# filrg/distributed_cluster_GPUs

Measured on AMD Instinct MI355X. Metric: sim_events_per_sec, higher is better.
Workload: dtype fp64; 1 GPU; model=paper_config multi-DC geo-cluster DES, global_batch=4096, seq_len=4000, parallelism=replica_shard_dp1, algo=default_policy, replicas_per_gpu=4096, arrivals=sinusoid inf 6/s amp 0.6 period 300 + poisson trn 0.3/s, fp32_coeff_eval=False, topology=8 DC / 1488 GPUs / 8 ingresses

## Files before the change

distributed_cluster_gpus_amd/engine/batched.py:

```python
import math
import os
from typing import Optional

import numpy as np
import torch

from ..models.arrivals import ArrivalProcess
from ..models.scenario import Scenario
from ..ops import load_sim_hip
from ..utils.csvlog import ClusterLogWriter, JobLogWriter
from ..utils.timers import ThroughputMeter
from .oracle import ALGOS
from .state import (INF, RL_HID, SERIES_METRICS, alloc_state, engine_cfg,
                    engine_dims, load_tensors)

SERIES_FLEET = "ALL"


class BatchedEngine:
    def __init__(self, scenario: Scenario,
                 arrival_inf: ArrivalProcess, arrival_trn: ArrivalProcess,
                 *, algo: str = "default_policy", replicas: int = 4096,
                 duration: float = 3600.0, log_interval: float = 10.0,
                 out_dir: Optional[str] = None, seed: int = 42,
                 power_cap: float = 0.0, control_interval: float = 5.0,
                 elastic_scaling: bool = False, eco_objective: str = "energy",
                 num_fixed_gpus: int = 1, fixed_freq: Optional[float] = None,
                 logger=None, show_progress: bool = False,
                 device: Optional[torch.device] = None,
# ... 1 lines not shown
                 tcap: int = 64, qcap: int = 24576,
                 events_per_launch: int = 50000,
                 enable_logs: bool = True,
                 sla_p99_ms: float = 500.0, energy_budget_j=None,
                 rl_device: str = 'cuda', rl_batch: int = 256,
                 rl_warmup: int = 1000, rl_buffer: int = 200000,
                 rl_train_interval: int = 256, rl_agent=None,
                 rl_stats_interval: int = 100,
                 rl_serve: str = "device", rl_deterministic: bool = False,
                 rl_exact_p99: bool = False, fp32_coeff_eval: bool = False,
                 rl_tr_limit: Optional[int] = None, rl_reserve_cus: int = 16,
                 rl_target_updates_per_s: float = 180.0,
                 tr_cap: int = 262144, arrival_trace=None,
                 subwave: int = 64,
                 pop_series: bool = False, pop_series_every: int = 1,
                 **_unused):
        if algo not in ALGOS:
            raise ValueError(f"unknown algo {algo!r}")
        if pop_series and int(pop_series_every) < 1:
            raise ValueError("pop_series_every must be >= 1")
        if not torch.cuda.is_available():
            raise RuntimeError("BatchedEngine requires a ROCm GPU "
                               "(no silent CPU fallback)")
        self._mod = load_sim_hip("_sim_hip" if subwave == 64 else "_sim_hip_mw")
        self.sc = scenario
        self.algo = algo
        self.device = device or torch.device("cuda", torch.cuda.current_device())
        self.end_time = float(duration)
        self.log_interval = float(log_interval)
        self.events_per_launch = int(events_per_launch)
# ... 67 lines not shown
                and not self._rl_det

        dims = engine_dims(
            scenario, algo=algo, n_rep=R, duration=duration,
            log_interval=log_interval, tcap=tcap, qcap=qcap,
            events_per_launch=events_per_launch,
            log_replica=self.log_replica,
            pop_series_every=self.pop_series_every,
            arrival_trace=arrival_trace, power_cap=power_cap,
            eco_objective=eco_objective, fp32_coeff_eval=fp32_coeff_eval,
            num_fixed_gpus=num_fixed_gpus, fixed_freq=fixed_freq, seed=seed,
            rep_id_offset=shard.start, sla_p99_ms=sla_p99_ms, tr_cap=tr_cap,
            elastic_scaling=elastic_scaling, rl_exact_p99=rl_exact_p99,
            serve_device=self._serve_device, weights_buffer=self._mfma_serve,
            rl_deterministic=rl_deterministic, rl_tr_limit=rl_tr_limit,
            rl_train_interval=rl_train_interval)
        self.dims = dims
        if self.pop_series:
            ps_bytes = dims.ps_cap * (n_dc + 1) * len(SERIES_METRICS) * R * 8
            import logging
            from ..utils.logging import LOGGER_NAME
            (logger or logging.getLogger(LOGGER_NAME)).info(
                f"pop_series: sample buffer {dims.ps_cap} ticks x {n_dc + 1} "
                f"rows x {len(SERIES_METRICS)} metrics x {R} replicas x 8 B = "
                f"{ps_bytes} bytes ({ps_bytes / 2**20:.1f} MiB)")
        t = alloc_state(dims, scenario, dev, arrival_trace)
        if not self.trace_mode:
            arr_np = self._seed_arrivals(arrival_inf, arrival_trn, seed, shard)
            t["arr_next"].copy_(torch.as_tensor(arr_np, dtype=torch.float64))
        self.t = t
        self.arrival_inf, self.arrival_trn = arrival_inf, arrival_trn
# ... 501 lines not shown
```

distributed_cluster_gpus_amd/engine/state.py:

```python
import math
from dataclasses import dataclass
from typing import Optional

import numpy as np
import torch

from ..models.scenario import PAYLOAD_GB, Scenario

ALGO_IDS = {"default_policy": 0, "cap_uniform": 1, "cap_greedy": 2,
            "joint_nf": 3, "bandit": 4, "carbon_cost": 5, "eco_route": 6,
            "debug": 7, "chsac_af": 8}
ECO_IDS = {"energy": 0, "carbon": 1, "cost": 2}
MODE_IDS = {"poisson": 0, "sinusoid": 1, "off": 2}
INF = 1e300
SERIES_METRICS = ("freq", "busy", "running", "q_inf", "q_trn", "power_w",
                  "energy_j")
RL_HID = 256
P99_WIN = 2048


@dataclass(frozen=True)
class EngineDims:
    algo: str
    n_rep: int
    n_dc: int
    n_ing: int
    n_freq: int
    total_slots: int
    tcap: int
    qcap: int
    end_time: float
    log_interval: float
    log_replica: int
# ... 8 lines not shown
    fp32_score: int
    num_fixed: int
    fixed_freq: float
    seed: int
    rep_id_offset: int
    sla_p99_ms: float
    obs_dim: int
    tr_cap: int
    pp_cap: int
    elastic: int
    exact_p99: int
    serve_device: int
    weights_numel: int
    rl_det: int
    tr_limit: int

    @property
    def is_rl(self) -> bool:
        return self.algo == "chsac_af"

    @property
    def n_streams(self) -> int:
        return self.n_ing * 2


def policy_weights_numel(obs_dim: int, n_dc: int, n_g: int,
                         hid: int = RL_HID) -> int:
    H = hid
    return (obs_dim * H + H) + 2 * (H * H + H) + (H * H + H) + \
        (H * n_dc + n_dc) + (H * H + H) + (H * n_g + n_g)


def engine_dims(scenario: Scenario, *, algo: str, n_rep: int,
                duration: float = 3600.0, log_interval: float = 10.0,
                tcap: int = 64, qcap: int = 24576,
                events_per_launch: int = 50000, log_replica: int = -1,
                pop_series_every: int = 0, arrival_trace=None,
                power_cap: float = 0.0, eco_objective: str = "energy",
                fp32_coeff_eval: bool = False, num_fixed_gpus: int = 1,
                fixed_freq: Optional[float] = None, seed: int = 42,
                rep_id_offset: int = 0, sla_p99_ms: float = 500.0,
                tr_cap: int = 262144, elastic_scaling: bool = False,
                rl_exact_p99: bool = False, serve_device: bool = False,
                weights_buffer: bool = False, rl_deterministic: bool = False,
                rl_tr_limit: Optional[int] = None,
                rl_train_interval: int = 256) -> EngineDims:
    is_rl = algo == "chsac_af"
    n_dc = scenario.n_dc
    end_time, log_interval = float(duration), float(log_interval)
    n_ticks = int(math.ceil(end_time / log_interval))
    logs = log_replica >= 0
    obs_dim = 1 + 6 * n_dc
    n_g = int(scenario.policy.max_gpus_per_job)
    tr_cap = int(tr_cap) if is_rl else 0
    tr_limit = int(rl_tr_limit) if rl_tr_limit is not None else \
        min(tr_cap // 2, int(rl_train_interval) * 256)
    return EngineDims(
        algo=algo, n_rep=int(n_rep), n_dc=n_dc, n_ing=scenario.n_ing,
        n_freq=scenario.n_freq,
        total_slots=int(scenario.total_gpus.sum()), tcap=int(tcap),
        qcap=int(qcap), end_time=end_time, log_interval=log_interval,
        log_replica=int(log_replica),
        cl_cap=(n_dc * (n_ticks + 2) + 64) if logs else 1,
        jl_cap=max(65536, 2 * int(events_per_launch)) if logs else 1,
        ps_every=int(pop_series_every),
        ps_cap=(n_ticks // int(pop_series_every) + 2) if pop_series_every
        else 0,
        trace_mode=arrival_trace is not None,
        trace_cap=int(np.asarray(arrival_trace[0]).shape[2])
        if arrival_trace is not None else 0,
        power_cap=float(power_cap), eco_obj=ECO_IDS[eco_objective],
        fp32_score=int(bool(fp32_coeff_eval)), num_fixed=int(num_fixed_gpus),
        fixed_freq=float(fixed_freq) if fixed_freq else 0.0,
        seed=int(seed), rep_id_offset=int(rep_id_offset),
        sla_p99_ms=float(sla_p99_ms),
        obs_dim=obs_dim, tr_cap=tr_cap,
        pp_cap=int(scenario.total_gpus.max()) if is_rl else 0,
        elastic=int(bool(elastic_scaling) and is_rl),
        exact_p99=int(bool(rl_exact_p99) and is_rl),
        serve_device=int(bool(serve_device) and is_rl),
        weights_numel=policy_weights_numel(obs_dim, n_dc, n_g)
        if (is_rl and (serve_device or weights_buffer)) else 1,
        rl_det=int(bool(rl_deterministic) and is_rl),
        tr_limit=tr_limit if is_rl else 0)


def alloc_state(dims: EngineDims, scenario: Scenario, device,
                arrival_trace=None) -> dict:
    d = dims
    dev = torch.device(device)
    R, n_dc, n_freq, NS = d.n_rep, d.n_dc, d.n_freq, d.n_streams
    total_slots, tcap, qcap = d.total_slots, d.tcap, d.qcap
    f64 = dict(dtype=torch.float64, device=dev)
    f32 = dict(dtype=torch.float32, device=dev)
    i64 = dict(dtype=torch.int64, device=dev)
    i32 = dict(dtype=torch.int32, device=dev)
    i16 = dict(dtype=torch.int16, device=dev)
    i8 = dict(dtype=torch.int8, device=dev)
    u8 = dict(dtype=torch.uint8, device=dev)
# ... 71 lines not shown
    t["jobs_done_inf"] = torch.zeros(R, **i64)
    t["sum_lat"] = torch.zeros(R, **f64)
    t["sum_lat_inf"] = torch.zeros(R, **f64)
    t["sum_wait"] = torch.zeros(R, **f64)
    t["cl_count"] = torch.zeros(1, **i32)
    t["cl_rows"] = torch.zeros((d.cl_cap, 15), **f64)
    t["jl_count"] = torch.zeros(1, **i32)
    t["jl_rows"] = torch.zeros((d.jl_cap, 11), **f64)

    if d.ps_every:
        t["ps_samples"] = torch.zeros(
            (d.ps_cap, n_dc + 1, len(SERIES_METRICS), R), **f64)
        t["ps_time"] = torch.zeros(d.ps_cap, **f64)
        t["ps_tick"] = torch.zeros(R, **i32)

    if d.trace_mode:
        tt, ts = arrival_trace[0], arrival_trace[1]
        td = arrival_trace[2] if len(arrival_trace) > 2 else \
            np.full(np.asarray(tt).shape, -1, np.int8)
        tt = np.asarray(tt, np.float64)
        ts = np.asarray(ts, np.float64)
        td = np.asarray(td, np.int8)
        assert tt.shape == (R, NS, d.trace_cap), tt.shape
        t["trace_time"] = T(tt)
        t["trace_size"] = T(ts)
        t["trace_dc"] = T(td)
        t["trace_pos"] = torch.zeros((R, NS), **i32)
        t["arr_next"].copy_(t["trace_time"][:, :, 0])

    if d.is_rl:
# ... 83 lines not shown
        "fp32_score": d.fp32_score, "num_fixed": d.num_fixed,
        "fixed_freq": d.fixed_freq,
        "payload_inf_gb": PAYLOAD_GB[0], "payload_trn_gb": PAYLOAD_GB[1],
        "arr_mode": [MODE_IDS[arrival_inf.mode], MODE_IDS[arrival_trn.mode]],
        "arr_rate": [float(arrival_inf.rate), float(arrival_trn.rate)],
        "arr_amp": [float(arrival_inf.amp), float(arrival_trn.amp)],
        "arr_period": [float(arrival_inf.period), float(arrival_trn.period)],
        "seed": d.seed, "rep_id_offset": d.rep_id_offset,
        "log_replica": d.log_replica, "cl_cap": d.cl_cap, "jl_cap": d.jl_cap,
        "obs_dim": d.obs_dim, "sla_p99_ms": d.sla_p99_ms, "tr_cap": d.tr_cap,
        "elastic": d.elastic, "pp_cap": d.pp_cap,
        "trace_mode": int(d.trace_mode), "trace_cap": d.trace_cap,
        "serve_device": d.serve_device, "rl_hid": RL_HID, "rl_det": d.rl_det,
        "tr_limit": d.tr_limit, "exact_p99": d.exact_p99,
        "p99_win": P99_WIN, "pop_series_every": d.ps_every,
    }
```

distributed_cluster_gpus_amd/ops/csrc/hip/engine_bind.hpp:

```cpp
#pragma once
#include <torch/extension.h>

#include <string>
#include <tuple>
#include <type_traits>
#include <unordered_map>
#include <vector>

#include "engine_desc.hpp"

namespace dcg {

template <class T> struct ElemOf;
#define DCG_ELEM(T, ST) \
  template <> struct ElemOf<T> { static constexpr auto dtype = torch::ST; }
DCG_ELEM(double, kFloat64);
DCG_ELEM(float, kFloat32);
DCG_ELEM(int, kInt32);
DCG_ELEM(short, kInt16);
DCG_ELEM(char, kInt8);
DCG_ELEM(unsigned char, kUInt8);
DCG_ELEM(long long, kInt64);
DCG_ELEM(uint64_t, kInt64);
DCG_ELEM(SRec, kFloat64);
DCG_ELEM(XRec, kFloat64);
#undef DCG_ELEM

class Binder {
 public:
  using Row = std::tuple<std::string, std::string, int64_t>;

  explicit Binder(const std::unordered_map<std::string, torch::Tensor>& t)
      : t_(t) {}

  template <class P>
  void operator()(P*& field, const char* name, int64_t need) {
    using E = std::remove_const_t<P>;
    const auto dtype = ElemOf<E>::dtype;
    const int64_t item = (int64_t)c10::elementSize(dtype);
    const int64_t per = (int64_t)sizeof(E) / item;
// ... 45 lines not shown
```

distributed_cluster_gpus_amd/ops/csrc/hip/engine_desc.hpp:

```cpp
#pragma once
#include <cstddef>
#include <cstdint>

namespace dcg {

constexpr int MAX_DC = 8;
constexpr int MAX_FREQ = 8;

struct XRec {
  double size;
  float netlat;
  int jid;
  short nsel;
  unsigned char dc, jtype, ing, adc, ag, mdc;
  unsigned char mg, has_rl, pad0, pad1;
};
static_assert(sizeof(XRec) == 32, "XRec must be one 32B record");

struct SRec {
  double start, lastupd, size, fused, done;
  float netlat;
  int jid;
  int seq;
  unsigned char ing, pcount, nrew, adc, ag, mdc, mg, has_rl;
  unsigned char pad[4];
};
static_assert(sizeof(SRec) == 64, "SRec must be one 64B record");

enum Algo { A_DEFAULT = 0, A_CAP_UNIFORM, A_CAP_GREEDY, A_JOINT_NF, A_BANDIT,
            A_CARBON_COST, A_ECO_ROUTE, A_DEBUG, A_CHSAC };

enum PendKind : int { PEND_NONE = 0, PEND_ARRIVAL = 1, PEND_DRAIN = 2,
                      PEND_REALLOC = 3 };
enum ReqFlag : int { REQ_IDLE = 0, REQ_PENDING = 1, REQ_READY = 2 };

constexpr int LAT_BINS = 64;

enum Err : int { ERR_NONE = 0, ERR_QUEUE_OVF = 1, ERR_XFER_OVF = 2,
                 ERR_SLOT_OVF = 4, ERR_LOG_OVF = 8 };

constexpr int MAX_STREAMS = 16;
constexpr int RL_MAX_HID = 256;
constexpr int RL_MAX_OBS = 64;
constexpr int RL_MAX_LOG = 16;

struct EngineDesc {
  int n_rep, n_dc, n_ing, n_freq, n_streams, total_slots, tcap, qcap;
  double end_time, log_interval;
  const double* freq_levels;
  const double* pc;
  const double* lc;
  const double* wan_lat;
  const double* wan_bw;
  const double* carbon;
// ... 119 lines not shown
  int p99_win;
  double* p99_sorted;
  double* p99_ring;
  int tr_cap;
  int* tr_count;
  float* tr_s0;
  float* tr_s1;
  unsigned char* tr_adc;
  unsigned char* tr_ag;
  float* tr_r;
  float* tr_costs;
  unsigned char* tr_mdc;
  unsigned char* tr_mg;
};

static_assert(sizeof(SRec) == 8 * sizeof(double), "s_rec rows are 8 f64 wide");
static_assert(sizeof(XRec) == 4 * sizeof(double), "x_rec rows are 4 f64 wide");

}
```

distributed_cluster_gpus_amd/ops/csrc/hip/replica_engine.hip:

```cpp
#include <torch/extension.h>
#include <ATen/hip/HIPContext.h>
#include <hip/hip_runtime.h>

#include <cstdint>
#include <cstdlib>
#include <string>
#include <tuple>
#include <unordered_map>
#include <vector>

#include "engine_bind.hpp"
#include "engine_desc.hpp"
#include "engine_limits.hpp"
#include "launch_plan.hpp"
#include "philox.hpp"
#include "pop_series.hpp"
#include "sim_models.hpp"

namespace dcg {

__device__ __forceinline__ void store_fence() {
  asm volatile("s_waitcnt vmcnt(0) lgkmcnt(0)" ::: "memory");
}

__device__ __forceinline__ void lds_fence() {
// ... 337 lines not shown

__device__ double draw_interarrival(Ctx& c, int jt, double t) {
  const EngineDesc& S = *c.S;
  double rate = S.arr_rate[jt];
  int mode = S.arr_mode[jt];
  double amp = S.arr_amp[jt];
  double period = S.arr_period[jt];
  double ia = D_INF;
  if (mode == 0 && rate > 0) {
    ia = rexp(c.rng, rate);
  } else if (mode == 1) {
    double max_rate = rate * (1.0 + fabs(amp));
    if (max_rate > 0) {
      for (int it = 0; it < 4096; ++it) {
        double w = rexp(c.rng, max_rate);
        double lam = fmax(0.0, rate * (1.0 + amp *
            sin(2.0 * M_PI * fmod(t + w, period) / period)));
        if (u01(c.rng) <= lam / max_rate) { ia = w; break; }
      }
    }
  }
  return ia;
}

__device__ void push_transfer(Ctx& c, double now, int jt, int ing, double size,
                              int jid, int d_sel,
                              const JobTrace* tr = nullptr) {
  const EngineDesc& S = *c.S;
  double lnet = launch_const(S.wan_lat)[ing * S.n_dc + d_sel];
  double bw = launch_const(S.wan_bw)[ing * S.n_dc + d_sel];
  double xfer = bw > 0.0 ? S.payload_gb[jt] / bw : 0.0;
  int cand = sub_first_empty(c.l_xt, 0, S.tcap);
// ... 698 lines not shown
    rl_serve_inline(c, now, a_dc, a_g, mdc, mg);
    rl_realloc_entry(c, cur, a_g, mdc, mg, now);
  }
  if (c.lane == 0) {
    S.pp_count[c.r] = 0;
    S.pp_cursor[c.r] = 0;
  }
  store_fence();
}

#if DCG_SUBWAVE == 8
#define DCG_ADVANCE_BOUNDS __launch_bounds__(THREADS_PER_BLOCK, 2)
#else
#define DCG_ADVANCE_BOUNDS __launch_bounds__(THREADS_PER_BLOCK)
#endif
template <int ALGO, bool PS, bool WIN>
__global__ void DCG_ADVANCE_BOUNDS
advance_kernel(EngineDesc S, double t_target, long long max_ev,
               PopSeriesDesc P, LaunchWindow W) {
  int slot_id = sub_uniform_i32((blockIdx.x * blockDim.x + threadIdx.x) / SUBW);
  int lane = threadIdx.x & (SUBW - 1);
  static_assert(!(WIN && ALGO == A_CHSAC), "chsac has no windowed kernel");
  if (slot_id >= (WIN ? W.count : S.n_rep)) return;
  long long ev_skip = 0;
  if (WIN) {
    slot_id += W.first;
    if (slot_id >= S.n_rep) slot_id -= S.n_rep;
    slot_id = sub_uniform_i32(slot_id);
    ev_skip = sub_uniform_i64(
        (blockIdx.x * blockDim.x + threadIdx.x) / SUBW >= W.split
            ? W.ev_a - W.ev_b : 0ll);
  }

  Ctx c;
  c.S = &S;
  c.r = slot_id;
  c.lane = lane;
  if (S.done[c.r]) return;
  if (ALGO == A_CHSAC && S.pend_kind[c.r] != PEND_NONE &&
      S.req_flag[c.r] != REQ_READY)
    return;
  c.now = S.now[c.r];
  {
    bool own = lane < S.n_dc;
    c.my_total = own ? S.total_gpus[lane] : 0;
    c.my_pidle = own ? (S.power_gating[lane] ? S.p_sleep[lane]
                                             : S.p_idle[lane]) : 0.0;
  }
  c.rng.key = S.seed ^ (0x9E3779B97F4A7C15ull * (uint64_t)(S.rep_id_offset + c.r));
  c.rng.ctr = S.rng_ctr[c.r];

  const int NS = S.n_streams;
  int64_t sbase = (int64_t)c.r * S.total_slots;
  long long n_events = ev_skip;
  bool paused = false;
  bool skip_loop = false;

  extern __shared__ __attribute__((aligned(16))) char smem[];
  {
    const LdsSizes z = lds_sizes(S.total_slots, S.tcap, ALGO == A_CHSAC);
    char* base = smem + (threadIdx.x / SUBW) * z.stride();
    c.hs = reinterpret_cast<Hot*>(base);
    if (SUBW == 64) {
      c.l_fin = reinterpret_cast<double*>(base + z.hot);
      c.l_xt = reinterpret_cast<double*>(base + z.hot + z.fin);
// ... 160 lines not shown
      break;
    }
    if (t_min > t_target) break;

    accrue_to(c, t_min);
    c.now = t_min;
    n_events++;

    if (kind == 0) {
      int ing = idx >> 1;
      int jt = idx & 1;
      int jid = c.hs->jid_ctr + 1;
      if (lane == 0) c.hs->jid_ctr = jid;
      double size;
      int trace_d = -1;
      if (S.trace_mode) {
        int64_t tb = ((int64_t)c.r * S.n_streams + idx) * S.trace_cap;
        int posn = S.trace_pos[(int64_t)c.r * S.n_streams + idx];
        size = S.trace_size[tb + posn];
        trace_d = S.trace_dc[tb + posn];
        int nxt = posn + 1;
        double t_next = nxt < S.trace_cap ? S.trace_time[tb + nxt] : D_INF;
        if (lane == 0) {
          S.trace_pos[(int64_t)c.r * S.n_streams + idx] = nxt;
          c.hs->arr_next[idx] = t_next;
        }
        lds_fence();
      } else {
        size = jt == 0 ? rpareto_inf(c.rng)
                       : fmax(0.1, rlognormal(c.rng, log(50000.0), 0.4));
      }
// ... 3 lines not shown
        if (lane == 0 && !S.trace_mode) c.hs->arr_next[idx] = t_min + ia_rl;
        lds_fence();
        if (S.serve_device) {
          int a_dc, a_g, mdc, mg;
          rl_serve_inline(c, t_min, a_dc, a_g, mdc, mg);
          JobTrace tr{c.l_obs, a_dc, a_g, mdc, mg, a_g + 1};
          push_transfer(c, t_min, jt, ing, size, jid, a_dc, &tr);
        } else {
          rl_request(c, PEND_ARRIVAL, t_min, jt, ing, size, 0.0f, jid,
                     -1, 0, t_min);
          paused = true;
          break;
        }
      } else {
      int d_sel;
      if (S.trace_mode && trace_d >= 0) {
        d_sel = trace_d;
      } else if (ALGO == A_ECO_ROUTE) {
        double price = S.eco_obj == 2 ? c.price_kwh(t_min) : 0.0;
        if (SUBW == 64) {
          double score = D_INF;
          {
            int d = lane >> 3;
            int n = (lane & 7) + 1;
            if (d < S.n_dc && n <= S.max_gpj) {
              kc_f64 pcf = c.pc3(d, jt);
              kc_f64 tcf = c.lc3(d, jt);
              double best = D_INF;
              for (int q = 0; q < S.n_freq; ++q) {
                double f = S.freq_levels[q];
                double T = d_unit_time(n, f, tcf);
// ... 31 lines not shown
                else if (S.eco_obj == 2) sc = (E / 3.6e6) * price;
                else sc = E;
                if (sc < best) best = sc;
              }
            score = best * size;
          }
          int dl;
          wave_argmin_f64(score, dl);
          d_sel = dl & (SUBW - 1);
        }
      } else {
        d_sel = (int)rbelow(c.rng, (uint32_t)S.n_dc);
      }
      d_sel = sub_uniform_i32(d_sel);
      push_transfer(c, t_min, jt, ing, size, jid, d_sel);
      double ia = D_INF;
      if (!S.trace_mode) ia = draw_interarrival(c, jt, t_min);
      if (lane == 0 && !S.trace_mode) c.hs->arr_next[idx] = t_min + ia;
      lds_fence();
      }

    } else if (kind == 1) {
      int64_t at = (int64_t)c.r * S.tcap + idx;
      XRec xr = S.x_rec[at];
      int d = sub_uniform_i32(xr.dc);
      int jt = sub_uniform_i32(xr.jtype);
      double size = xr.size;
      float netlat = xr.netlat;
      int jid = xr.jid;
      int ing = xr.ing;
      if (lane == 0) c.l_xt[idx] = D_INF;
      lds_fence();
      if (c.free_gpus(d) > 0) {
        if (ALGO == A_CHSAC && xr.has_rl) {
// ... 156 lines not shown
      S.acc_unit[rd] = h->acc_unit[lane];
      S.util_begin[rd] = h->util_begin[lane];
      S.cur_freq[rd] = h->cur_freq[lane];
      S.busy[rd] = h->busy[lane];
      S.n_running[rd] = h->n_running[lane];
    }
    for (int k = lane; k < nd * 2; k += SUBW) {
      S.q_len[c.r * nd * 2 + k] = h->q_len[k];
      S.q_head[c.r * nd * 2 + k] = h->q_head[k];
    }
  }
  if (lane == 0) {
    S.next_log[c.r] = c.hs->next_log;
    S.now[c.r] = c.now;
    S.rng_ctr[c.r] = c.rng.ctr;
    S.ev_count[c.r] += n_events - ev_skip;
    S.sum_lat[c.r] = c.hs->sum_lat;
    S.sum_lat_inf[c.r] = c.hs->sum_lat_inf;
    S.sum_wait[c.r] = c.hs->sum_wait;
    S.jobs_done[c.r] = c.hs->jobs_done;
    S.jobs_done_inf[c.r] = c.hs->jobs_done_inf;
    S.jid_ctr[c.r] = c.hs->jid_ctr;
    S.seq_ctr[c.r] = c.hs->seq_ctr;
  }
}


constexpr int MF_STRIDE = 257;
using mf_acc = __attribute__((ext_vector_type(4))) float;

// ... 164 lines not shown
    auto ar = cfg["arr_rate"].cast<std::vector<double>>();
    auto aa = cfg["arr_amp"].cast<std::vector<double>>();
    auto ap = cfg["arr_period"].cast<std::vector<double>>();
    for (int j = 0; j < 2; ++j) {
      S_.arr_mode[j] = am[j]; S_.arr_rate[j] = ar[j];
      S_.arr_amp[j] = aa[j]; S_.arr_period[j] = ap[j];
    }
    S_.seed = cfg["seed"].cast<uint64_t>();
    S_.rep_id_offset = cfg["rep_id_offset"].cast<int64_t>();
    S_.log_replica = cfg["log_replica"].cast<int>();
    S_.cl_cap = cfg["cl_cap"].cast<int>();
    S_.jl_cap = cfg["jl_cap"].cast<int>();

    S_.trace_mode = opt("trace_mode", 0);
    S_.trace_cap = opt("trace_cap", 0);
    S_.obs_dim = opt("obs_dim", 0);
    S_.sla_p99_ms = opt("sla_p99_ms", 500.0);
    S_.tr_cap = opt("tr_cap", 0);
    S_.elastic = opt("elastic", 0);
    S_.pp_cap = opt("pp_cap", 0);
    S_.serve_device = opt("serve_device", 0);
    S_.hid = opt("rl_hid", 256);
    S_.n_g = S_.max_gpj;
    S_.rl_det = opt("rl_det", 0);
    S_.tr_limit = opt("tr_limit", 0);
    if (S_.algo == A_CHSAC) {
      S_.exact_p99 = opt("exact_p99", 0);
      S_.p99_win = opt("p99_win", 2048);
    }
    ps_.every = opt("pop_series_every", 0);
// ... 66 lines not shown
    bind(S_.jobs_done, "jobs_done", R);
    bind(S_.jobs_done_inf, "jobs_done_inf", R);
    bind(S_.sum_lat, "sum_lat", R);
    bind(S_.sum_lat_inf, "sum_lat_inf", R);
    bind(S_.sum_wait, "sum_wait", R);
    bind(S_.cl_count, "cl_count", 1);
    bind(S_.cl_rows, "cl_rows", (int64_t)S_.cl_cap * 15);
    bind(S_.jl_count, "jl_count", 1);
    bind(S_.jl_rows, "jl_rows", (int64_t)S_.jl_cap * 11);
    if (S_.trace_mode) {
      bind(S_.trace_time, "trace_time", R * NS * S_.trace_cap);
      bind(S_.trace_size, "trace_size", R * NS * S_.trace_cap);
      bind(S_.trace_dc, "trace_dc", R * NS * S_.trace_cap);
      bind(S_.trace_pos, "trace_pos", R * NS);
    }
    if (S_.serve_device) {
      const int64_t H = S_.hid, G = S_.n_g;
      bind(S_.pw, "policy_weights",
           (O * H + H) + 2 * (H * H + H) + (H * H + H) + (H * D + D) +
               (H * H + H) + (H * G + G));
    }
    if (S_.algo == A_CHSAC) {
      const int64_t PP = S_.pp_cap, TR = S_.tr_cap;
      bind(S_.req_flag, "req_flag", R);
      bind(S_.req_obs, "req_obs", R * O);
      bind(S_.req_mdc, "req_mdc", R);
      bind(S_.req_mg, "req_mg", R);
      bind(S_.resp_dc, "resp_dc", R);
      bind(S_.resp_g, "resp_g", R);
      bind(S_.pend_kind, "pend_kind", R);
// ... 124 lines not shown
          reinterpret_cast<const void*>(kernel(S_.algo != A_CHSAC)),
          THREADS_PER_BLOCK,
          shmem_bytes());
      if (e == hipSuccess) e = hipGetDevice(&dev);
      if (e == hipSuccess)
        e = hipDeviceGetAttribute(&n_cu, hipDeviceAttributeMultiprocessorCount,
                                  dev);
      if (e != hipSuccess || per_cu < 1 || n_cu < 1)
        throw std::runtime_error(std::string("advance occupancy query: ") +
                                 hipGetErrorString(e));
      queried_capacity_ = per_cu * n_cu * REPLICAS_PER_BLOCK;
    }
    return queried_capacity_;
  }

  LaunchPlan plan_for(long long max_ev) {
    if (max_passes_ <= 1 || S_.algo == A_CHSAC || masked_stream_) {
      LaunchPlan p;
      p.windows.push_back(single_window(S_.n_rep, max_ev));
      return p;
    }
    return make_launch_plan(S_.n_rep, resident_capacity(), max_ev,
                            max_passes_, min_quantum_, launch_cost_);
  }

  std::vector<std::tuple<int, int, int, int64_t, int64_t>> launch_plan(
      int64_t max_ev) {
    std::vector<std::tuple<int, int, int, int64_t, int64_t>> out;
    for (const LaunchWindow& w : plan_for(max_ev).windows)
      out.emplace_back(w.first, w.count, w.split, (int64_t)w.ev_a,
                       (int64_t)w.ev_b);
    return out;
  }

  void advance(double t_target, int64_t max_ev) {
    require_gpu("advance");
    const int rpb = REPLICAS_PER_BLOCK;
    const LaunchPlan plan = plan_for(max_ev);
    AdvanceFn fn = kernel(plan.windows.size() > 1);
    size_t shmem = shmem_bytes();
    dim3 block(THREADS_PER_BLOCK);
    for (const LaunchWindow& w : plan.windows) {
      dim3 grid((w.count + rpb - 1) / rpb);
      hipLaunchKernelGGL(fn, grid, block, shmem, stream(), S_, t_target,
                         w.ev_a, ps_, w);
      check_launch("advance_kernel launch failed");
    }
  }

 private:
  void require_gpu(const char* what) const {
    if (!on_gpu_)
      throw std::runtime_error(std::string(what) + ": the engine's tensors "
                               "are on " + device_ + ", not on a GPU");
  }

  hipStream_t stream() const {
    return masked_stream_ ? masked_stream_
                          : (hipStream_t)at::hip::getCurrentHIPStream();
  }

  using AdvanceFn = void (*)(EngineDesc, double, long long, PopSeriesDesc,
                             LaunchWindow);

  AdvanceFn kernel(bool windowed) const {
#define DCG_ADVANCE_ROW(PS, WIN, CHSAC)                                        \
  {advance_kernel<A_DEFAULT, PS, WIN>,    advance_kernel<A_CAP_UNIFORM, PS, WIN>, \
   advance_kernel<A_CAP_GREEDY, PS, WIN>, advance_kernel<A_JOINT_NF, PS, WIN>, \
   advance_kernel<A_BANDIT, PS, WIN>,     advance_kernel<A_CARBON_COST, PS, WIN>, \
   advance_kernel<A_ECO_ROUTE, PS, WIN>,  advance_kernel<A_DEBUG, PS, WIN>,    \
   CHSAC}
    static const AdvanceFn kernels[2][2][A_CHSAC + 1] = {
        {DCG_ADVANCE_ROW(false, false, (advance_kernel<A_CHSAC, false, false>)),
         DCG_ADVANCE_ROW(true, false, (advance_kernel<A_CHSAC, true, false>))},
        {DCG_ADVANCE_ROW(false, true, nullptr),
         DCG_ADVANCE_ROW(true, true, nullptr)}};
#undef DCG_ADVANCE_ROW
    if (S_.algo < 0 || S_.algo > A_CHSAC)
      throw std::runtime_error("unsupported algo for HIP engine");
    AdvanceFn fn = kernels[windowed][ps_.samples != nullptr][S_.algo];
    if (!fn) throw std::runtime_error("chsac has no windowed advance kernel");
    return fn;
  }

  size_t shmem_bytes() const {
    size_t shmem = REPLICAS_PER_BLOCK *
                   lds_sizes(S_.total_slots, S_.tcap,
                             S_.algo == A_CHSAC).stride();
    if (shmem > 64 * 1024)
      throw std::runtime_error(
          "scenario too large for the LDS-mirrored engine (total_slots = " +
          std::to_string(S_.total_slots) + " + tcap = " +
          std::to_string(S_.tcap) + " need " + std::to_string(shmem) +
          " B, above the 64 KiB dynamic-LDS budget per block)");
    return shmem;
  }

  EngineDesc S_{};
  PopSeriesDesc ps_{};
  int forced_capacity_ = 0;
  int queried_capacity_ = 0;
  int max_passes_ = PLAN_MAX_PASSES;
  long long min_quantum_ = PLAN_MIN_QUANTUM;
  long long launch_cost_ = PLAN_LAUNCH_COST;
  std::unordered_map<std::string, torch::Tensor> t_;
  std::vector<Binder::Row> contract_;
  bool on_gpu_ = false;
  std::string device_;
  hipStream_t masked_stream_ = nullptr;
};

}

PYBIND11_MODULE(TORCH_EXTENSION_NAME, m) {
// ... 2 lines not shown
      .def(py::init<py::dict, py::dict>())
      .def("advance", &dcg::BatchedSimHip::advance,
           py::arg("t_target"), py::arg("max_events"))
      .def("set_launch_plan", &dcg::BatchedSimHip::set_launch_plan,
           "resident_capacity 0 = query the runtime; max_passes 1 = single "
           "launch; min_quantum, launch_cost (events) < 0 = defaults",
           py::arg("resident_capacity"), py::arg("max_passes"),
           py::arg("min_quantum") = -1, py::arg("launch_cost") = -1)
      .def("launch_plan", &dcg::BatchedSimHip::launch_plan,
           "windows (first, count, split, ev_a, ev_b) advance() would launch",
           py::arg("max_events"))
      .def("contract", &dcg::BatchedSimHip::contract,
           "bound tensors in bind order: (field, dtype, required numel; -1 = "
           "never dereferenced in this configuration)")
      .def("resident_capacity", &dcg::BatchedSimHip::resident_capacity)
      .def("enable_masked_stream", &dcg::BatchedSimHip::enable_masked_stream,
           py::arg("n_reserved_cus"))
      .def("masked_active", &dcg::BatchedSimHip::masked_active)
      .def("advance_done", &dcg::BatchedSimHip::advance_done)
      .def("advance_sync", &dcg::BatchedSimHip::advance_sync);
  m.def("reduce_series", &dcg::reduce_series,
        "population time-series reduction (samples[T,C,R] f64, ticks[R] i32, "
        "every) -> stats[T,C,5] f64 = {n, mean, M2, min, max}; replica r "
        "counts at tick t iff ticks[r] / every > t",
        py::arg("samples"), py::arg("ticks"), py::arg("every"));
  m.def("rl_forward_mfma", &dcg::rl_forward_mfma,
        "MFMA (matrix-core) batched actor forward "
        "(pw, obs[B,D], hid, n_dc, n_g) -> (logits_dc, logits_g)",
        py::arg("pw"), py::arg("obs"), py::arg("hid"), py::arg("n_dc"),
        py::arg("n_g"));
// ... 3 lines not shown
```

Before: 620.5 million events/s.

## Pre-generate arrivals into a per-replica ring with a cooperative 8-lane kernel

```diff
diff --git a/distributed_cluster_gpus_amd/engine/batched.py b/distributed_cluster_gpus_amd/engine/batched.py
--- a/distributed_cluster_gpus_amd/engine/batched.py
+++ b/distributed_cluster_gpus_amd/engine/batched.py
@@ -11,8 +11,8 @@
 from ..utils.csvlog import ClusterLogWriter, JobLogWriter
 from ..utils.timers import ThroughputMeter
 from .oracle import ALGOS
-from .state import (INF, RL_HID, SERIES_METRICS, alloc_state, engine_cfg,
-                    engine_dims, load_tensors)
+from .state import (ARR_CAP, INF, RL_HID, SERIES_METRICS, alloc_state,
+                    engine_cfg, engine_dims, load_tensors)
 
 SERIES_FLEET = "ALL"
 
@@ -44,6 +44,7 @@
                  tr_cap: int = 262144, arrival_trace=None,
                  subwave: int = 64,
                  pop_series: bool = False, pop_series_every: int = 1,
+                 arrival_pregen: bool = True, arr_cap: int = ARR_CAP,
                  **_unused):
         if algo not in ALGOS:
             raise ValueError(f"unknown algo {algo!r}")
@@ -141,7 +142,9 @@
             elastic_scaling=elastic_scaling, rl_exact_p99=rl_exact_p99,
             serve_device=self._serve_device, weights_buffer=self._mfma_serve,
             rl_deterministic=rl_deterministic, rl_tr_limit=rl_tr_limit,
-            rl_train_interval=rl_train_interval)
+            rl_train_interval=rl_train_interval,
+            arrival_pregen=bool(arrival_pregen) and subwave == 64,
+            arr_cap=arr_cap)
         self.dims = dims
         if self.pop_series:
             ps_bytes = dims.ps_cap * (n_dc + 1) * len(SERIES_METRICS) * R * 8
diff --git a/distributed_cluster_gpus_amd/engine/state.py b/distributed_cluster_gpus_amd/engine/state.py
--- a/distributed_cluster_gpus_amd/engine/state.py
+++ b/distributed_cluster_gpus_amd/engine/state.py
@@ -17,6 +17,7 @@
                   "energy_j")
 RL_HID = 256
 P99_WIN = 2048
+ARR_CAP = 4096
 
 
 @dataclass(frozen=True)
@@ -55,6 +56,7 @@
     weights_numel: int
     rl_det: int
     tr_limit: int
+    arr_cap: int = 0
 
     @property
     def is_rl(self) -> bool:
@@ -85,7 +87,9 @@
                 rl_exact_p99: bool = False, serve_device: bool = False,
                 weights_buffer: bool = False, rl_deterministic: bool = False,
                 rl_tr_limit: Optional[int] = None,
-                rl_train_interval: int = 256) -> EngineDims:
+                rl_train_interval: int = 256,
+                arrival_pregen: bool = True,
+                arr_cap: int = ARR_CAP) -> EngineDims:
     is_rl = algo == "chsac_af"
     n_dc = scenario.n_dc
     end_time, log_interval = float(duration), float(log_interval)
@@ -96,6 +100,9 @@
     tr_cap = int(tr_cap) if is_rl else 0
     tr_limit = int(rl_tr_limit) if rl_tr_limit is not None else \
         min(tr_cap // 2, int(rl_train_interval) * 256)
+    pregen = bool(arrival_pregen) and not is_rl and arrival_trace is None
+    if pregen and (int(arr_cap) < 1 or int(arr_cap) & (int(arr_cap) - 1)):
+        raise ValueError(f"arr_cap must be a power of two, got {arr_cap}")
     return EngineDims(
         algo=algo, n_rep=int(n_rep), n_dc=n_dc, n_ing=scenario.n_ing,
         n_freq=scenario.n_freq,
@@ -123,7 +130,8 @@
         weights_numel=policy_weights_numel(obs_dim, n_dc, n_g)
         if (is_rl and (serve_device or weights_buffer)) else 1,
         rl_det=int(bool(rl_deterministic) and is_rl),
-        tr_limit=tr_limit if is_rl else 0)
+        tr_limit=tr_limit if is_rl else 0,
+        arr_cap=int(arr_cap) if pregen else 0)
 
 
 def alloc_state(dims: EngineDims, scenario: Scenario, device,
@@ -225,6 +233,14 @@
         t["ps_time"] = torch.zeros(d.ps_cap, **f64)
         t["ps_tick"] = torch.zeros(R, **i32)
 
+    if d.arr_cap:
+        t["arr_ring"] = torch.zeros((R, d.arr_cap, 4), **f64)
+        t["arr_head"] = torch.zeros(R, **i32)
+        t["arr_count"] = torch.zeros(R, **i32)
+        t["gen_arr_next"] = torch.full((R, NS), INF, **f64)
+        t["gen_ctr"] = torch.zeros(R, **i64)
+        t["arr_more"] = torch.zeros(1, **i32)
+
     if d.trace_mode:
         tt, ts = arrival_trace[0], arrival_trace[1]
         td = arrival_trace[2] if len(arrival_trace) > 2 else \
@@ -338,4 +354,5 @@
         "serve_device": d.serve_device, "rl_hid": RL_HID, "rl_det": d.rl_det,
         "tr_limit": d.tr_limit, "exact_p99": d.exact_p99,
         "p99_win": P99_WIN, "pop_series_every": d.ps_every,
+        "arr_cap": d.arr_cap,
     }
diff --git a/distributed_cluster_gpus_amd/ops/csrc/hip/arrival_plan.hpp b/distributed_cluster_gpus_amd/ops/csrc/hip/arrival_plan.hpp
--- /dev/null
+++ b/distributed_cluster_gpus_amd/ops/csrc/hip/arrival_plan.hpp
@@ -0,0 +1,31 @@
+#pragma once
+
+#if defined(__HIPCC__) || defined(__CUDACC__)
+#define DCG_HD __host__ __device__
+#else
+#define DCG_HD
+#endif
+
+namespace dcg {
+
+DCG_HD inline bool arr_cap_valid(long long cap) {
+  return cap >= 1 && cap <= (1ll << 30) && (cap & (cap - 1)) == 0;
+}
+
+DCG_HD inline int ring_slot(int head, int i, int cap) {
+  return (int)(((long long)head + i) & (cap - 1));
+}
+
+DCG_HD inline long long ring_topup_target(long long budget, long long cap) {
+  if (budget < 0) budget = 0;
+  return budget < cap ? budget : cap;
+}
+
+DCG_HD inline int substep_count(long long E, long long cap) {
+  return E <= 0 ? 1 : (int)((E + cap - 1) / cap);
+}
+DCG_HD inline long long substep_budget(long long E, int n, int i) {
+  return E <= 0 ? E : E / n + (i < E % n ? 1 : 0);
+}
+
+}
diff --git a/distributed_cluster_gpus_amd/ops/csrc/hip/arrival_ring.hpp b/distributed_cluster_gpus_amd/ops/csrc/hip/arrival_ring.hpp
--- /dev/null
+++ b/distributed_cluster_gpus_amd/ops/csrc/hip/arrival_ring.hpp
@@ -0,0 +1,163 @@
+#pragma once
+#include <hip/hip_runtime.h>
+
+#include <cmath>
+#include <cstdint>
+
+#include "arrival_plan.hpp"
+#include "engine_desc.hpp"
+#include "philox.hpp"
+#include "sim_models.hpp"
+
+namespace dcg {
+
+__device__ __forceinline__ double thinning_rate(double rate, double amp,
+                                                double period, double t,
+                                                double w) {
+  return fmax(0.0, rate * (1.0 + amp *
+      sin(2.0 * M_PI * fmod(t + w, period) / period)));
+}
+
+__device__ __forceinline__ double job_size_map(int jt, double ua, double ub) {
+  return jt == 0 ? rpareto_inf_map(ua)
+                 : fmax(0.1, rlognormal_map(ua, ub, log(50000.0), 0.4));
+}
+
+#if DCG_SUBWAVE == 64
+constexpr int PG_GROUP = 8;
+constexpr int PG_THREADS = 256;
+static_assert(MAX_STREAMS == 2 * PG_GROUP, "two stream times per lane");
+
+__device__ __forceinline__ int pg_group_ballot(bool p, int lane64) {
+  unsigned long long m = __ballot(p);
+  return (int)((m >> (lane64 & ~(PG_GROUP - 1))) & 0xffull);
+}
+
+__global__ void __launch_bounds__(PG_THREADS)
+pregen_arrivals_kernel(EngineDesc S, ArrRing A, double t_target,
+                       long long budget) {
+  const int r = (int)((blockIdx.x * (unsigned)PG_THREADS + threadIdx.x) /
+                      PG_GROUP);
+  const int gl = threadIdx.x & (PG_GROUP - 1);
+  const int lane64 = threadIdx.x & 63;
+  const int NS = S.n_streams;
+  const bool live = r < S.n_rep && !S.done[r];
+  const long long target = ring_topup_target(budget, A.cap);
+  const double t_lim = fmin(S.end_time, t_target);
+  const int n_hdr = S.algo == A_ECO_ROUTE ? 1 : 2;
+
+  int count = 0, head = 0;
+  uint64_t ctr = 0, key = 0;
+  double s0 = D_INF, s1 = D_INF;
+  if (live) {
+    count = A.count[r];
+    head = A.head[r];
+    const bool empty = count == 0;
+    const double* an = (empty ? S.arr_next : A.gen_arr_next) + (int64_t)r * NS;
+    ctr = empty ? S.rng_ctr[r] : A.gen_ctr[r];
+    if (2 * gl < NS) s0 = an[2 * gl];
+    if (2 * gl + 1 < NS) s1 = an[2 * gl + 1];
+    key = S.seed ^ (0x9E3779B97F4A7C15ull * (uint64_t)(S.rep_id_offset + r));
+  }
+
+  bool pend = false;
+  uint64_t p_ctr = 0, p_after = 0;
+  double p_tnext = 0.0;
+  int p_stream = 0, p_slot = 0;
+  auto flush = [&]() {
+    if (pend) {
+      uint32_t w[4];
+      philox4x32(key, p_ctr, w);
+      double ua = u01_map(w[0], w[1]);
+      double ub = ((w[2] >> 5) * 67108864.0 + (w[3] >> 6)) *
+                  (1.0 / 9007199254740992.0);
+      ARec rec;
+      rec.size = job_size_map(p_stream & 1, ua, ub);
+      rec.t_next = p_tnext;
+      rec.ctr = p_after;
+      rec.stream = p_stream;
+      rec.dc = -1;
+      if (n_hdr == 2) {
+        philox4x32(key, p_ctr + 1, w);
+        rec.dc = (int)rbelow_map(w[0], (uint32_t)S.n_dc);
+      }
+      A.ring[(int64_t)r * A.cap + p_slot] = rec;
+      pend = false;
+    }
+  };
+
+  bool act = live;
+  for (int it = 0;; ++it) {
+    if (act) act = count < target;
+    double bv = s0;
+    int bi = 2 * gl;
+    if (act) {
+      if (s1 < bv) { bv = s1; bi = 2 * gl + 1; }
+#pragma unroll
+      for (int off = 1; off < PG_GROUP; off <<= 1) {
+        double ov = __shfl_xor(bv, off, 64);
+        int oi = __shfl_xor(bi, off, 64);
+        if (ov < bv || (ov == bv && oi < bi)) { bv = ov; bi = oi; }
+      }
+      if (bv > t_lim) act = false;
+    }
+    if (!__any(act)) break;
+    if (act) {
+      const int jt = bi & 1;
+      const uint64_t c_hdr = ctr;
+      uint64_t c = ctr + n_hdr;
+      const double rate = jt ? S.arr_rate[1] : S.arr_rate[0];
+      const int mode = jt ? S.arr_mode[1] : S.arr_mode[0];
+      const double amp = jt ? S.arr_amp[1] : S.arr_amp[0];
+      const double period = jt ? S.arr_period[1] : S.arr_period[0];
+      const double lambd = mode == 1 ? rate * (1.0 + fabs(amp)) : rate;
+      double ia = D_INF;
+      if ((mode == 0 || mode == 1) && lambd > 0) {
+        for (int pass = 0; pass < 4096 / (PG_GROUP / 2); ++pass) {
+          uint32_t w[4];
+          philox4x32(key, c + (mode == 1 ? gl : 0), w);
+          double u = u01_map(w[0], w[1]);
+          double wv = rexp_map(u, lambd);
+          if (mode == 0) { ia = wv; c += 1; break; }
+          double thr = thinning_rate(rate, amp, period, bv, wv) / lambd;
+          double un = __shfl_down(u, 1, 64);
+          int m = pg_group_ballot(!(gl & 1) && un <= thr, lane64);
+          if (m) {
+            int first = __ffs(m) - 1;
+            ia = __shfl(wv, (lane64 & ~(PG_GROUP - 1)) + first, 64);
+            c += first + 2;
+            break;
+          }
+          c += PG_GROUP;
+        }
+      }
+      const double tn = bv + ia;
+      if (bi == 2 * gl) s0 = tn;
+      if (bi == 2 * gl + 1) s1 = tn;
+      ctr = c;
+      if ((it & (PG_GROUP - 1)) == gl) {
+        pend = true;
+        p_ctr = c_hdr;
+        p_after = c;
+        p_tnext = tn;
+        p_stream = bi;
+        p_slot = ring_slot(head, count, A.cap);
+      }
+      ++count;
+    }
+    if ((it & (PG_GROUP - 1)) == PG_GROUP - 1) flush();
+  }
+  flush();
+
+  if (live) {
+    if (2 * gl < NS) A.gen_arr_next[(int64_t)r * NS + 2 * gl] = s0;
+    if (2 * gl + 1 < NS) A.gen_arr_next[(int64_t)r * NS + 2 * gl + 1] = s1;
+    if (gl == 0) {
+      A.gen_ctr[r] = ctr;
+      A.count[r] = count;
+    }
+  }
+}
+#endif
+
+}
diff --git a/distributed_cluster_gpus_amd/ops/csrc/hip/engine_bind.hpp b/distributed_cluster_gpus_amd/ops/csrc/hip/engine_bind.hpp
--- a/distributed_cluster_gpus_amd/ops/csrc/hip/engine_bind.hpp
+++ b/distributed_cluster_gpus_amd/ops/csrc/hip/engine_bind.hpp
@@ -24,6 +24,7 @@
 DCG_ELEM(uint64_t, kInt64);
 DCG_ELEM(SRec, kFloat64);
 DCG_ELEM(XRec, kFloat64);
+DCG_ELEM(ARec, kFloat64);
 #undef DCG_ELEM
 
 class Binder {
diff --git a/distributed_cluster_gpus_amd/ops/csrc/hip/engine_desc.hpp b/distributed_cluster_gpus_amd/ops/csrc/hip/engine_desc.hpp
--- a/distributed_cluster_gpus_amd/ops/csrc/hip/engine_desc.hpp
+++ b/distributed_cluster_gpus_amd/ops/csrc/hip/engine_desc.hpp
@@ -27,6 +27,15 @@
 };
 static_assert(sizeof(SRec) == 64, "SRec must be one 64B record");
 
+struct ARec {
+  double size;
+  double t_next;
+  uint64_t ctr;
+  int stream;
+  int dc;
+};
+static_assert(sizeof(ARec) == 32, "ARec must be one 32B record");
+
 enum Algo { A_DEFAULT = 0, A_CAP_UNIFORM, A_CAP_GREEDY, A_JOINT_NF, A_BANDIT,
             A_CARBON_COST, A_ECO_ROUTE, A_DEBUG, A_CHSAC };
 
@@ -37,7 +46,8 @@
 constexpr int LAT_BINS = 64;
 
 enum Err : int { ERR_NONE = 0, ERR_QUEUE_OVF = 1, ERR_XFER_OVF = 2,
-                 ERR_SLOT_OVF = 4, ERR_LOG_OVF = 8 };
+                 ERR_SLOT_OVF = 4, ERR_LOG_OVF = 8,
+                 ERR_ARR_RING = 16 };
 
 constexpr int MAX_STREAMS = 16;
 constexpr int RL_MAX_HID = 256;
@@ -187,7 +197,18 @@
   unsigned char* tr_mg;
 };
 
+struct ArrRing {
+  int cap;
+  ARec* ring;
+  int* head;
+  int* count;
+  double* gen_arr_next;
+  uint64_t* gen_ctr;
+  int* more;
+};
+
 static_assert(sizeof(SRec) == 8 * sizeof(double), "s_rec rows are 8 f64 wide");
 static_assert(sizeof(XRec) == 4 * sizeof(double), "x_rec rows are 4 f64 wide");
+static_assert(sizeof(ARec) == 4 * sizeof(double), "arr_ring rows are 4 f64 wide");
 
 }
diff --git a/distributed_cluster_gpus_amd/ops/csrc/hip/replica_engine.hip b/distributed_cluster_gpus_amd/ops/csrc/hip/replica_engine.hip
--- a/distributed_cluster_gpus_amd/ops/csrc/hip/replica_engine.hip
+++ b/distributed_cluster_gpus_amd/ops/csrc/hip/replica_engine.hip
@@ -9,6 +9,7 @@
 #include <unordered_map>
 #include <vector>
 
+#include "arrival_ring.hpp"
 #include "engine_bind.hpp"
 #include "engine_desc.hpp"
 #include "engine_limits.hpp"
@@ -376,8 +377,7 @@
     if (max_rate > 0) {
       for (int it = 0; it < 4096; ++it) {
         double w = rexp(c.rng, max_rate);
-        double lam = fmax(0.0, rate * (1.0 + amp *
-            sin(2.0 * M_PI * fmod(t + w, period) / period)));
+        double lam = thinning_rate(rate, amp, period, t, w);
         if (u01(c.rng) <= lam / max_rate) { ia = w; break; }
       }
     }
@@ -1106,13 +1106,15 @@
 #else
 #define DCG_ADVANCE_BOUNDS __launch_bounds__(THREADS_PER_BLOCK)
 #endif
-template <int ALGO, bool PS, bool WIN>
+template <int ALGO, bool PS, bool WIN, bool PRE = false>
 __global__ void DCG_ADVANCE_BOUNDS
 advance_kernel(EngineDesc S, double t_target, long long max_ev,
-               PopSeriesDesc P, LaunchWindow W) {
+               PopSeriesDesc P, LaunchWindow W, ArrRing A) {
   int slot_id = sub_uniform_i32((blockIdx.x * blockDim.x + threadIdx.x) / SUBW);
   int lane = threadIdx.x & (SUBW - 1);
   static_assert(!(WIN && ALGO == A_CHSAC), "chsac has no windowed kernel");
+  static_assert(!(PRE && (ALGO == A_CHSAC || SUBW != 64)),
+                "chsac draws at its arrivals; the 8-lane build has no ring");
   if (slot_id >= (WIN ? W.count : S.n_rep)) return;
   long long ev_skip = 0;
   if (WIN) {
@@ -1141,6 +1143,11 @@
   }
   c.rng.key = S.seed ^ (0x9E3779B97F4A7C15ull * (uint64_t)(S.rep_id_offset + c.r));
   c.rng.ctr = S.rng_ctr[c.r];
+  int ring_head = 0, ring_left = 0;
+  if (PRE) {
+    ring_head = sub_uniform_i32(A.head[c.r]);
+    ring_left = sub_uniform_i32(A.count[c.r]);
+  }
 
   const int NS = S.n_streams;
   int64_t sbase = (int64_t)c.r * S.total_slots;
@@ -1331,7 +1338,19 @@
       if (lane == 0) c.hs->jid_ctr = jid;
       double size;
       int trace_d = -1;
-      if (S.trace_mode) {
+      if (PRE) {
+        ARec rec = A.ring[(int64_t)c.r * A.cap + ring_head];
+        if (ring_left <= 0 || sub_uniform_i32(rec.stream) != idx) {
+          if (lane == 0) atomicOr(&S.err[c.r], ERR_ARR_RING);
+        }
+        size = rec.size;
+        trace_d = sub_uniform_i32(rec.dc);
+        c.rng.ctr = (uint64_t)sub_uniform_i64((long long)rec.ctr);
+        ring_head = ring_slot(ring_head, 1, A.cap);
+        --ring_left;
+        if (lane == 0) c.hs->arr_next[idx] = rec.t_next;
+        lds_fence();
+      } else if (S.trace_mode) {
         int64_t tb = ((int64_t)c.r * S.n_streams + idx) * S.trace_cap;
         int posn = S.trace_pos[(int64_t)c.r * S.n_streams + idx];
         size = S.trace_size[tb + posn];
@@ -1365,7 +1384,7 @@
         }
       } else {
       int d_sel;
-      if (S.trace_mode && trace_d >= 0) {
+      if ((PRE || S.trace_mode) && trace_d >= 0) {
         d_sel = trace_d;
       } else if (ALGO == A_ECO_ROUTE) {
         double price = S.eco_obj == 2 ? c.price_kwh(t_min) : 0.0;
@@ -1427,10 +1446,12 @@
       }
       d_sel = sub_uniform_i32(d_sel);
       push_transfer(c, t_min, jt, ing, size, jid, d_sel);
+      if (!PRE) {
       double ia = D_INF;
       if (!S.trace_mode) ia = draw_interarrival(c, jt, t_min);
       if (lane == 0 && !S.trace_mode) c.hs->arr_next[idx] = t_min + ia;
       lds_fence();
+      }
       }
 
     } else if (kind == 1) {
@@ -1617,6 +1638,11 @@
     S.next_log[c.r] = c.hs->next_log;
     S.now[c.r] = c.now;
     S.rng_ctr[c.r] = c.rng.ctr;
+    if (PRE) {
+      A.head[c.r] = ring_head;
+      A.count[c.r] = max(ring_left, 0);
+      if (n_events >= max_ev) *A.more = 1;
+    }
     S.ev_count[c.r] += n_events - ev_skip;
     S.sum_lat[c.r] = c.hs->sum_lat;
     S.sum_lat_inf[c.r] = c.hs->sum_lat_inf;
@@ -1811,6 +1837,17 @@
 
     S_.trace_mode = opt("trace_mode", 0);
     S_.trace_cap = opt("trace_cap", 0);
+    ar_.cap = opt("arr_cap", 0);
+    if (ar_.cap != 0) {
+      if (!arr_cap_valid(ar_.cap))
+        throw std::invalid_argument(
+            "engine limits: arr_cap = " + std::to_string(ar_.cap) +
+            ", required a power of two");
+      if (S_.algo == A_CHSAC || S_.trace_mode)
+        throw std::invalid_argument(
+            "arr_cap = " + std::to_string(ar_.cap) + ": chsac_af and "
+            "trace mode have no pre-generated arrivals, required arr_cap = 0");
+    }
     S_.obs_dim = opt("obs_dim", 0);
     S_.sla_p99_ms = opt("sla_p99_ms", 500.0);
     S_.tr_cap = opt("tr_cap", 0);
@@ -1907,6 +1944,21 @@
       bind(S_.trace_dc, "trace_dc", R * NS * S_.trace_cap);
       bind(S_.trace_pos, "trace_pos", R * NS);
     }
+    if (ar_.cap > 0) {
+#if DCG_SUBWAVE == 64
+      bind(ar_.ring, "arr_ring", R * ar_.cap);
+      bind(ar_.head, "arr_head", R);
+      bind(ar_.count, "arr_count", R);
+      bind(ar_.gen_arr_next, "gen_arr_next", R * NS);
+      bind(ar_.gen_ctr, "gen_ctr", R);
+      bind(ar_.more, "arr_more", 1);
+#else
+      for (const char* n : {"arr_ring", "arr_head", "arr_count",
+                            "gen_arr_next", "gen_ctr", "arr_more"})
+        bind.unused(n);
+      ar_.cap = 0;
+#endif
+    }
     if (S_.serve_device) {
       const int64_t H = S_.hid, G = S_.n_g;
       bind(S_.pw, "policy_weights",
@@ -2061,6 +2113,13 @@
     return queried_capacity_;
   }
 
+  std::vector<long long> substeps(long long max_ev) const {
+    std::vector<long long> out;
+    const int n = ar_.cap > 0 ? substep_count(max_ev, ar_.cap) : 1;
+    for (int i = 0; i < n; ++i) out.push_back(substep_budget(max_ev, n, i));
+    return out;
+  }
+
   LaunchPlan plan_for(long long max_ev) {
     if (max_passes_ <= 1 || S_.algo == A_CHSAC || masked_stream_) {
       LaunchPlan p;
@@ -2074,26 +2133,61 @@
   std::vector<std::tuple<int, int, int, int64_t, int64_t>> launch_plan(
       int64_t max_ev) {
     std::vector<std::tuple<int, int, int, int64_t, int64_t>> out;
-    for (const LaunchWindow& w : plan_for(max_ev).windows)
-      out.emplace_back(w.first, w.count, w.split, (int64_t)w.ev_a,
-                       (int64_t)w.ev_b);
+    for (long long ev : substeps(max_ev))
+      for (const LaunchWindow& w : plan_for(ev).windows)
+        out.emplace_back(w.first, w.count, w.split, (int64_t)w.ev_a,
+                         (int64_t)w.ev_b);
     return out;
   }
 
   void advance(double t_target, int64_t max_ev) {
     require_gpu("advance");
     const int rpb = REPLICAS_PER_BLOCK;
-    const LaunchPlan plan = plan_for(max_ev);
-    AdvanceFn fn = kernel(plan.windows.size() > 1);
     size_t shmem = shmem_bytes();
     dim3 block(THREADS_PER_BLOCK);
-    for (const LaunchWindow& w : plan.windows) {
-      dim3 grid((w.count + rpb - 1) / rpb);
-      hipLaunchKernelGGL(fn, grid, block, shmem, stream(), S_, t_target,
-                         w.ev_a, ps_, w);
-      check_launch("advance_kernel launch failed");
-    }
-  }
+    const std::vector<long long> subs = substeps(max_ev);
+    for (size_t i = 0; i < subs.size(); ++i) {
+      const long long ev = subs[i];
+      if (subs.size() > SUBSTEP_CHECK && i % SUBSTEP_CHECK == 0) {
+        if (i > 0 && !budget_limited()) break;
+        hipError_t e = hipMemsetAsync(ar_.more, 0, sizeof(int), stream());
+        if (e != hipSuccess)
+          throw std::runtime_error(std::string("advance: ") +
+                                   hipGetErrorString(e));
+      }
+#if DCG_SUBWAVE == 64
+      if (ar_.cap > 0) {
+        const int per_block = PG_THREADS / PG_GROUP;
+        hipLaunchKernelGGL(pregen_arrivals_kernel,
+                           dim3((S_.n_rep + per_block - 1) / per_block),
+                           dim3(PG_THREADS), 0, stream(), S_, ar_, t_target,
+                           ev);
+        check_launch("pregen_arrivals_kernel launch failed");
+      }
+#endif
+      const LaunchPlan plan = plan_for(ev);
+      AdvanceFn fn = kernel(plan.windows.size() > 1);
+      for (const LaunchWindow& w : plan.windows) {
+        dim3 grid((w.count + rpb - 1) / rpb);
+        hipLaunchKernelGGL(fn, grid, block, shmem, stream(), S_, t_target,
+                           w.ev_a, ps_, w, ar_);
+        check_launch("advance_kernel launch failed");
+      }
+    }
+  }
+
+  bool budget_limited() {
+    int more = 1;
+    hipError_t e = hipMemcpyAsync(&more, ar_.more, sizeof(int),
+                                  hipMemcpyDeviceToHost, stream());
+    if (e == hipSuccess) e = hipStreamSynchronize(stream());
+    if (e != hipSuccess)
+      throw std::runtime_error(std::string("advance: ") +
+                               hipGetErrorString(e));
+    return more != 0;
+  }
+
+  bool arrival_pregen() const { return ar_.cap > 0; }
 
  private:
   void require_gpu(const char* what) const {
@@ -2108,24 +2202,42 @@
   }
 
   using AdvanceFn = void (*)(EngineDesc, double, long long, PopSeriesDesc,
-                             LaunchWindow);
+                             LaunchWindow, ArrRing);
 
   AdvanceFn kernel(bool windowed) const {
-#define DCG_ADVANCE_ROW(PS, WIN, CHSAC)                                        \
-  {advance_kernel<A_DEFAULT, PS, WIN>,    advance_kernel<A_CAP_UNIFORM, PS, WIN>, \
-   advance_kernel<A_CAP_GREEDY, PS, WIN>, advance_kernel<A_JOINT_NF, PS, WIN>, \
-   advance_kernel<A_BANDIT, PS, WIN>,     advance_kernel<A_CARBON_COST, PS, WIN>, \
-   advance_kernel<A_ECO_ROUTE, PS, WIN>,  advance_kernel<A_DEBUG, PS, WIN>,    \
+#define DCG_ADVANCE_ROW(PS, WIN, PRE, CHSAC)                                   \
+  {advance_kernel<A_DEFAULT, PS, WIN, PRE>,                                    \
+   advance_kernel<A_CAP_UNIFORM, PS, WIN, PRE>,                                \
+   advance_kernel<A_CAP_GREEDY, PS, WIN, PRE>,                                 \
+   advance_kernel<A_JOINT_NF, PS, WIN, PRE>,                                   \
+   advance_kernel<A_BANDIT, PS, WIN, PRE>,                                     \
+   advance_kernel<A_CARBON_COST, PS, WIN, PRE>,                                \
+   advance_kernel<A_ECO_ROUTE, PS, WIN, PRE>,                                  \
+   advance_kernel<A_DEBUG, PS, WIN, PRE>,                                      \
    CHSAC}
+#define DCG_ADVANCE_TABLE(PRE)                                                 \
+  {{DCG_ADVANCE_ROW(false, false, PRE, nullptr),                               \
+    DCG_ADVANCE_ROW(true, false, PRE, nullptr)},                               \
+   {DCG_ADVANCE_ROW(false, true, PRE, nullptr),                                \
+    DCG_ADVANCE_ROW(true, true, PRE, nullptr)}}
     static const AdvanceFn kernels[2][2][A_CHSAC + 1] = {
-        {DCG_ADVANCE_ROW(false, false, (advance_kernel<A_CHSAC, false, false>)),
-         DCG_ADVANCE_ROW(true, false, (advance_kernel<A_CHSAC, true, false>))},
-        {DCG_ADVANCE_ROW(false, true, nullptr),
-         DCG_ADVANCE_ROW(true, true, nullptr)}};
-#undef DCG_ADVANCE_ROW
+        {DCG_ADVANCE_ROW(false, false, false,
+                         (advance_kernel<A_CHSAC, false, false>)),
+         DCG_ADVANCE_ROW(true, false, false,
+                         (advance_kernel<A_CHSAC, true, false>))},
+        {DCG_ADVANCE_ROW(false, true, false, nullptr),
+         DCG_ADVANCE_ROW(true, true, false, nullptr)}};
     if (S_.algo < 0 || S_.algo > A_CHSAC)
       throw std::runtime_error("unsupported algo for HIP engine");
     AdvanceFn fn = kernels[windowed][ps_.samples != nullptr][S_.algo];
+#if DCG_SUBWAVE == 64
+    static const AdvanceFn pre_kernels[2][2][A_CHSAC + 1] =
+        DCG_ADVANCE_TABLE(true);
+    if (ar_.cap > 0)
+      fn = pre_kernels[windowed][ps_.samples != nullptr][S_.algo];
+#endif
+#undef DCG_ADVANCE_TABLE
+#undef DCG_ADVANCE_ROW
     if (!fn) throw std::runtime_error("chsac has no windowed advance kernel");
     return fn;
   }
@@ -2143,8 +2255,10 @@
     return shmem;
   }
 
+  static constexpr size_t SUBSTEP_CHECK = 8;
   EngineDesc S_{};
   PopSeriesDesc ps_{};
+  ArrRing ar_{};
   int forced_capacity_ = 0;
   int queried_capacity_ = 0;
   int max_passes_ = PLAN_MAX_PASSES;
@@ -2177,6 +2291,9 @@
            "bound tensors in bind order: (field, dtype, required numel; -1 = "
            "never dereferenced in this configuration)")
       .def("resident_capacity", &dcg::BatchedSimHip::resident_capacity)
+      .def("arrival_pregen", &dcg::BatchedSimHip::arrival_pregen,
+           "arrivals come from the pre-generated ring (false: drawn inside "
+           "the advance kernel)")
       .def("enable_masked_stream", &dcg::BatchedSimHip::enable_masked_stream,
            py::arg("n_reserved_cus"))
       .def("masked_active", &dcg::BatchedSimHip::masked_active)
```

Measured after the change: 718.2 million events/s, median of 6. 15.8% higher.
